# Raph1821/Matcha-TTS-etu-UPMC-ENSAM

Hardware: AMD Instinct MI355X
Metric: training utterances/sec (whole node) + maximum_path Mcells/sec, LJSpeech batch=32 (higher is better)
Workload: dtype bf16; 1 GPU; MatchaTTS train step (encoder + MAS + CFM decoder fwd/bwd + clip + AdamW), B=32/GPU, Tx=120, Ty=600, 80 mels; model=MatchaTTS(n_vocab=150, out_channels=80, hidden_channels=192), global_batch=32, seq_len=600, text_len=120, parallelism=dp1, precision=bf16-parity, hip_graph=True, weight_planes=2, text_encoder_forward=fp32fwd (backward bf16)

## Files before the change

include/mtts_decoder.h:

```cpp
#ifndef MTTS_DECODER_H_
#define MTTS_DECODER_H_

#include <stddef.h>
#include <stdint.h>

#ifdef __cplusplus
extern "C" {
#endif

#define MTTS_PREC_FP32 0
#define MTTS_PREC_BF16 1

#define MTTS_ACT_NONE 0
#define MTTS_ACT_GELU 1
#define MTTS_ACT_DGELU 2
#define MTTS_ACT_RELU 3
#define MTTS_ACT_DRELU 4

#define MTTS_CONV_MAX_TAPS 8
#define MTTS_GEMM_GLDS 32
#define MTTS_GEMM_WREG 96

typedef struct mtts_conv_gemm_args {
    const float *A;
// ... 22 lines not shown
#define MTTS_GEMM_F_A_BF16 0x2
#define MTTS_GEMM_F_C_BF16 0x4
#define MTTS_GEMM_F_FAST_ACT 0x8
#define MTTS_GEMM_F_PRE_BF16 0x10
#define MTTS_GEMM_F_W_SPLIT 0x40
#define MTTS_GEMM_F_A_SPLIT 0x80

#define MTTS_GEMM_F_SPLIT3 0x100

int mtts_conv_gemm(const mtts_conv_gemm_args *args, int32_t precision, void *hip_stream);
int mtts_conv_gemm_tile(const mtts_conv_gemm_args *args, int32_t precision, int32_t tile_cfg, void *hip_stream);
size_t mtts_conv_gemm_workspace_size(const mtts_conv_gemm_args *args, int32_t precision, int32_t tile_cfg,
                                     int32_t splits);
int mtts_conv_gemm_ws(const mtts_conv_gemm_args *args, int32_t precision, int32_t tile_cfg, int32_t splits,
                      void *workspace, size_t workspace_bytes, void *hip_stream);

typedef struct mtts_conv_wgrad_args {
    const float *dY;
    int32_t ldy, To_full, out_stride, out_off;
    const float *A;
    const float *a_scale;
    int32_t lda, Ti, To, nb, in_stride, ntaps;
    int32_t off[MTTS_CONV_MAX_TAPS];
    int32_t cin;
    int32_t N, K;
    int32_t flags;
} mtts_conv_wgrad_args;
#define MTTS_WGRAD_F_DY_BF16 0x20

size_t mtts_conv_wgrad_workspace_size(const mtts_conv_wgrad_args *args);
// ... 155 lines not shown
```

matcha-tts-etu-upmc-ensam_amd/csrc/conv_gemm.hip:

```cpp
#include <hip/hip_runtime.h>

#include <algorithm>
#include <atomic>
#include <cstdio>
#include <cstdlib>
#include <mutex>
#include <vector>

#include <cstdint>

#include "gemm_epilogue.h"
#include "conv_gemm_wreg.h"
#include "mtts_common.h"
#include "mtts_decoder.h"

namespace {

typedef __bf16 bf16x8 __attribute__((ext_vector_type(8)));
typedef float f32x16 __attribute__((ext_vector_type(16)));
typedef short s16x4 __attribute__((ext_vector_type(4)));
typedef short s16x8 __attribute__((ext_vector_type(8)));

__device__ __forceinline__ bf16x8 tr_read8(const uint16_t *p, int row_stride) {
    using LdsS4 = __attribute__((address_space(3))) s16x4;
// ... 839 lines not shown
        case 9: launch_cfg<BF16, 9>(p, M, st, splits, part); break;
        case 10: launch_cfg<BF16, 10>(p, M, st, splits, part); break;
        case 11: launch_cfg<BF16, 11>(p, M, st, splits, part); break;
        case 12: launch_cfg<BF16, 12>(p, M, st, splits, part); break;
        case 13: launch_cfg<BF16, 13>(p, M, st, splits, part); break;
        case 14: launch_cfg<BF16, 14>(p, M, st, splits, part); break;
        case 15: launch_cfg<BF16, 15>(p, M, st, splits, part); break;
        case 16: launch_cfg<BF16, 16>(p, M, st, splits, part); break;
        case 17: launch_cfg<BF16, 17>(p, M, st, splits, part); break;
        default: launch_cfg<BF16, 18>(p, M, st, splits, part); break;
    }
}

static int glds_tiles(const mtts_conv_gemm_args &p, int M) { return ((M + 63) / 64) * ((p.N + 255) / 256); }

static int pick_cfg(const mtts_conv_gemm_args &p, int M, bool bf16) {
    static const int d2 = [] { const char *e = getenv("MTTS_GEMM_F32_DEPTH2"); return e ? (e[0] == '1' ? 1 : 0) : -1; }();
    if (!bf16) return M <= 8192 ? (d2 == 1 ? 18 : 3) : (d2 == 0 ? 7 : 11);
    if (p.act == MTTS_ACT_GELU || p.act == MTTS_ACT_DGELU) return 7;
    static const int sched_mask = [] {
        const char *e = getenv("MTTS_GEMM_SCHED_OFF");
        return e ? atoi(e) : 0;
    }();
    if ((sched_mask & 4) && mtts::conv_gemm_glds_applies(p) && p.K >= 512) {
        const int t = ((M + 127) / 128) * ((p.N + 255) / 256);
        if (t >= 128 && t <= 256) return MTTS_GEMM_GLDS + 14;
    }
    if (!(sched_mask & 2) && mtts::conv_gemm_glds_applies(p) && p.K >= 768) {
        const int t = glds_tiles(p, M);
        if ((t >= 128 && t <= 256) || (t < 128 && p.K >= 1536 && p.N % 4 == 0)) return MTTS_GEMM_GLDS + 10;
        if (!(sched_mask & 8) && t > 256 && mtts::conv_gemm_glds_lean(p)) return MTTS_GEMM_GLDS + 13;
    }
    if (!(sched_mask & 8) && p.K < 768 && p.N >= 512 && glds_tiles(p, M) >= 256 && mtts::conv_gemm_glds_applies(p) &&
        mtts::conv_gemm_glds_lean(p))
        return MTTS_GEMM_GLDS + 9;
    return p.K >= 384 ? 12 : 7;
}

static int pick_cfg_a16(const mtts_conv_gemm_args &p, int M) {
    if (p.act == MTTS_ACT_GELU || p.act == MTTS_ACT_DGELU) return MTTS_GEMM_GLDS + 12;
    return glds_tiles(p, M) >= 256 ? MTTS_GEMM_GLDS + 9 : MTTS_GEMM_GLDS + 12;
}

static int pick_cfg_ws(const mtts_conv_gemm_args &p, int M) {
    if (p.act == MTTS_ACT_GELU || p.act == MTTS_ACT_DGELU) return 7;
    if (!mtts::conv_gemm_glds_applies(p) || !mtts::conv_gemm_glds_lean(p)) return 7;
    const bool big = M >= 16384 && p.N <= 256;
    if (p.flags & MTTS_GEMM_F_A_BF16) return big ? MTTS_GEMM_GLDS + 12 : MTTS_GEMM_GLDS + 9;
    return M >= 16384 ? MTTS_GEMM_GLDS + 13 : MTTS_GEMM_GLDS + 9;
}

static int pick_splits_f32(const mtts_conv_gemm_args &p, int M, int cfg, int splits) {
    static const bool off = [] { const char *e = getenv("MTTS_GEMM_F32_SPLITK"); return e && e[0] == '0'; }();
    if (p.N % 4 || off || !mtts::gemm_epilogue_vec_ok(p)) return 1;
    if (splits > 0) return splits;
    const int nk = (p.K + kBK - 1) / kBK;
    if (cfg == 3 || cfg == 18) {
        const int tiles = ((M + 63) / 64) * ((p.N + 63) / 64);
        if (tiles >= 256 || nk < 20) return 1;
        return nk >= 28 ? 4 : 2;
    }
    if (cfg != 7 && cfg != 11) return 1;
    const int tiles = ((M + 31) / 32) * ((p.N + 127) / 128);
    if (tiles >= 256 || nk < 16) return 1;
// ... 155 lines not shown
    return conv_gemm_impl(args, precision, -1, 1, nullptr, 0, hip_stream);
}

extern "C" int mtts_conv_gemm_tile(const mtts_conv_gemm_args *args, int32_t precision, int32_t tile_cfg,
                                   void *hip_stream) {
    return conv_gemm_impl(args, precision, tile_cfg, 1, nullptr, 0, hip_stream);
}

extern "C" size_t mtts_conv_gemm_workspace_size(const mtts_conv_gemm_args *args, int32_t precision, int32_t tile_cfg,
                                                int32_t splits) {
    if (!args || args->nb * args->To == 0) return 0;
    const bool bf16 = precision == MTTS_PREC_BF16;
    int rc = MTTS_OK;
    const int cfg = resolve_cfg(*args, bf16, tile_cfg, args->nb * args->To, &rc);
    return rc ? 0 : plan_gemm(*args, bf16, cfg, splits).ws;
}

extern "C" int mtts_conv_gemm_ws(const mtts_conv_gemm_args *args, int32_t precision, int32_t tile_cfg, int32_t splits,
                                 void *workspace, size_t workspace_bytes, void *hip_stream) {
    return conv_gemm_impl(args, precision, tile_cfg, splits, workspace, workspace_bytes, hip_stream);
}

__global__ void dropout_apply_kernel(const float *__restrict__ x, float *__restrict__ y, int rows, int cols, int ld,
                                     float p, const uint32_t *__restrict__ seed) {
    const int64_t idx = (int64_t)blockIdx.x * blockDim.x + threadIdx.x;
    if (idx >= (int64_t)rows * cols) return;
    const uint32_t s0 = seed[0], s1 = seed[1];
    const int r = (int)(idx / cols), c = (int)(idx - (int64_t)r * cols);
    const float v = x[(size_t)r * ld + c];
    y[(size_t)r * ld + c] = mtts::dropout_keep(s0, s1, (uint32_t)r, (uint32_t)c, p) ? v * mtts::dropout_scale(p) : 0.f;
// ... 341 lines not shown
```

matcha-tts-etu-upmc-ensam_amd/csrc/conv_gemm_glds.hip:

```cpp
#include <hip/hip_runtime.h>

#include <cstdint>
#include <type_traits>
#include <utility>

#include "gemm_epilogue.h"
#include "lds_dma.h"
#include "mtts_common.h"
#include "mtts_decoder.h"

namespace {

typedef __bf16 bf16x8 __attribute__((ext_vector_type(8)));
typedef float f32x2 __attribute__((ext_vector_type(2)));
typedef __bf16 bf16x2 __attribute__((ext_vector_type(2)));
using mtts::f32x16;

__device__ uint4 g_zero16 = {0u, 0u, 0u, 0u};

#ifndef MTTS_GEMM_TIMELINE
#define MTTS_GEMM_TIMELINE 0
#endif
#if MTTS_GEMM_TIMELINE
constexpr int kTlSlots = 128, kTlWaves = 16384, kTlSteps = 60;
// ... 12 lines not shown
constexpr int kBK = 64;

__device__ __forceinline__ uint32_t pack2(float a, float b) {
    return __builtin_bit_cast(uint32_t, __builtin_convertvector((f32x2){a, b}, bf16x2));
}

using mtts::bload16;
using mtts::glds16;
using mtts::make_rsrc;
using mtts::u32x4;
using mtts::wait_vmcnt;
constexpr uint32_t MTTS_GLDS_OOB = mtts::kDmaOob;

template <int WM, int WN, int TM, int TN, int STAGES, bool ABF16 = false, int NPL = 1>
struct GldsGeom {
    static constexpr int NT = 64 * WM * WN;
    static constexpr int BM = 32 * WM * TM, BN = 32 * WN * TN;
    static constexpr int A_BYTES = BM * kBK * (ABF16 ? 2 : 4);
    static constexpr int W_BYTES = NPL * BN * kBK * 2;
    static constexpr int GA = A_BYTES / (NT * 16);
    static constexpr int GW = W_BYTES / (NT * 16);
    static_assert(A_BYTES % (NT * 16) == 0 && W_BYTES % (NT * 16) == 0, "tile / threads mismatch");
};

template <int WM, int WN, int TM, int TN, int STAGES, bool ABF16, bool LEAN, bool WS = false, bool X3 = false>
__global__ __launch_bounds__(64 * WM * WN) void conv_gemm_glds_kernel(mtts_conv_gemm_args p, int ksteps, float *part) {
    static_assert(!X3 || (!ABF16 && !WS), "bf16x6: fp32 A, three weight planes");
    constexpr int NPL = X3 ? 3 : (WS ? 2 : 1);
    using G = GldsGeom<WM, WN, TM, TN, STAGES, ABF16, NPL>;
    constexpr int ES = ABF16 ? 2 : 4;
    constexpr int RPI = ABF16 ? 8 : 4;
    constexpr int CPR = ABF16 ? 8 : 16;
    constexpr int EPC = 16 / ES;
    constexpr int NT = G::NT, BM = G::BM, BN = G::BN, GA = G::GA, GW = G::GW, NW = NT / 64;
    __shared__ __attribute__((aligned(1024))) unsigned char sA0[G::A_BYTES], sW0[G::W_BYTES];
    __shared__ __attribute__((aligned(1024))) unsigned char sA1[G::A_BYTES], sW1[G::W_BYTES];
    __shared__ __attribute__((aligned(1024))) unsigned char sA2[STAGES > 2 ? G::A_BYTES : 16],
        sW2[STAGES > 2 ? G::W_BYTES : 16];
    auto abuf = [&](auto S) -> unsigned char * {
        if constexpr (decltype(S)::value == 0) return sA0;
        else if constexpr (decltype(S)::value == 1) return sA1;
        else return sA2;
    };
    auto wbuf = [&](auto S) -> unsigned char * {
        if constexpr (decltype(S)::value == 0) return sW0;
        else if constexpr (decltype(S)::value == 1) return sW1;
        else return sW2;
    };
    typedef __attribute__((address_space(3))) unsigned char lds_u8;
    auto lds_addr = [](const lds_u8 *q) { return (uint32_t)(uintptr_t)q; };
    auto abuf_l = [&](auto S) -> uint32_t {
        if constexpr (decltype(S)::value == 0) return lds_addr((const lds_u8 *)sA0);
        else if constexpr (decltype(S)::value == 1) return lds_addr((const lds_u8 *)sA1);
        else return lds_addr((const lds_u8 *)sA2);
    };
    auto wbuf_l = [&](auto S) -> uint32_t {
        if constexpr (decltype(S)::value == 0) return lds_addr((const lds_u8 *)sW0);
        else if constexpr (decltype(S)::value == 1) return lds_addr((const lds_u8 *)sW1);
        else return lds_addr((const lds_u8 *)sW2);
    };

    const int tid = threadIdx.x, lane = tid & 63;
    const int wave = __builtin_amdgcn_readfirstlane(tid >> 6);
    const int wr = wave / WN, wc = wave % WN;
    const int lr = lane & 31, lh = lane >> 5;
    const int M = p.nb * p.To;
    int m0, n0, kstep0 = 0, nk = (p.K + kBK - 1) / kBK;
    {
        const int nt = (p.N + BN - 1) / BN;
        const int ntiles = ((M + BM - 1) / BM) * nt;
        const int S = gridDim.x / ntiles;
        int t = mtts::xcd_relabel(blockIdx.x, gridDim.x);
        if (S > 1) {
            const int tile = t / S, split = t - tile * S;
            t = tile;
            kstep0 = split * ksteps;
            nk = min(ksteps, nk - kstep0);
        }
        const int mt = t / nt;
        m0 = mt * BM;
        n0 = (t - mt * nt) * BN;
// ... 72 lines not shown
            const int ni = 8 * (i * NW + wave) + (lane >> 3);
            const int pl = NPL > 1 ? ni / BN : 0;
            const int n = ni - pl * BN;
            const int lc = (lane & 7) ^ ((ni >> 1) & 7);
            l_vw[i] = w_nok[i] ? (uint32_t)((pl * w_plane + (size_t)(n0 + n) * p.Kp + lc * 8) * 2) : MTTS_GLDS_OOB;
        }
    }

    auto issue = [&](auto S) {
        unsigned char *abase = abuf(S);
        unsigned char *wbase = wbuf(S);
        if constexpr (LEAN) {
            const uint32_t la = abuf_l(S), lw = wbuf_l(S);
#pragma unroll
            for (int i = 0; i < GA; ++i)
                bload16(l_vo[i], l_rsa, l_soa, __builtin_amdgcn_readfirstlane(la + (i * NW + wave) * 1024));
#pragma unroll
            for (int i = 0; i < GW; ++i)
                bload16(l_vw[i], l_rsw, l_sow, __builtin_amdgcn_readfirstlane(lw + (i * NW + wave) * 1024));
            l_sow += kBK * 2;
            l_soa += kBK * ES;
            if (--l_chs == 0) {
                ++l_tap;
                l_chs = p.cin / kBK;
                l_soa = 0;
#pragma unroll
                for (int i = 0; i < GA; ++i)
                    l_vo[i] = ((a_ok[i] >> min(l_tap, 31)) & 1u) ? (uint32_t)((l_row[i] + l_tap * tapstride) * ES)
                                                                 : MTTS_GLDS_OOB;
            }
            return;
        }
#pragma unroll
        for (int i = 0; i < GA; ++i) {
            const bool ok = (a_ok[i] >> min(a_j[i], 31)) & 1u;
            glds16(ok ? static_cast<const void *>(a_src[i]) : static_cast<const void *>(zero),
                   abase + (i * NW + wave) * 1024);
            a_ch[i] += kBK;
            a_src[i] += kBK * ES;
            const bool w = a_ch[i] >= p.cin;
            a_ch[i] -= w ? p.cin : 0;
            a_j[i] += w;
            a_src[i] += w ? tap_delta : 0;
        }
#pragma unroll
        for (int i = 0; i < GW; ++i) {
            const bool ok = w_nok[i] && w_k[i] < p.Kp;
            glds16(ok ? static_cast<const void *>(w_ptr[i]) : static_cast<const void *>(zero),
                   wbase + (i * NW + wave) * 1024);
            w_ptr[i] += kBK;
            w_k[i] += kBK;
        }
    };

    f32x16 acc[TM][TN];
#pragma unroll
    for (int i = 0; i < TM; ++i)
#pragma unroll
        for (int j = 0; j < TN; ++j)
#pragma unroll
            for (int v = 0; v < 16; ++v) acc[i][j][v] = 0.f;

    auto compute = [&](auto S) {
        const unsigned char *abase = abuf(S);
// ... 89 lines not shown
#pragma unroll
                    for (int j = 0; j < TN; ++j)
                        acc[i][j] = __builtin_amdgcn_mfma_f32_32x32x16_bf16(af[i], bfr[j], acc[i][j], 0, 0, 0);
            }
        }
    };

#if MTTS_GEMM_TIMELINE
    if (lane == 0 && (int)blockIdx.x * NW + wave < kTlWaves)
        g_tlg[((int)blockIdx.x * NW + wave) * kTlSlots] =
            ((long long)__smid() << 32) | (long long)__builtin_amdgcn_s_getreg((31 << 11) | 4);
    MTTS_TLG(1);
#endif
    issue(std::integral_constant<int, 0>{});
    if constexpr (STAGES > 2) issue(std::integral_constant<int, 1>{});
    MTTS_TLG(2);
    int tl_k = 0;
    (void)tl_k;
    auto step = [&](auto S) {
        constexpr int cur = decltype(S)::value, nxt = (cur + STAGES - 1) % STAGES;
        wait_vmcnt<(GA + GW) * (STAGES - 2)>();
        mtts::lds_barrier();
#if MTTS_GEMM_TIMELINE
        if (tl_k < kTlSteps) MTTS_TLG(3 + 2 * tl_k);
#endif
        issue(std::integral_constant<int, nxt>{});
        compute(S);
#if MTTS_GEMM_TIMELINE
        __builtin_amdgcn_sched_barrier(0);
        if (tl_k < kTlSteps) MTTS_TLG(4 + 2 * tl_k);
        ++tl_k;
#endif
    };
    for (int kt = 0; kt < nk; kt += STAGES) {
        step(std::integral_constant<int, 0>{});
        if (kt + 1 >= nk) break;
        step(std::integral_constant<int, 1>{});
        if constexpr (STAGES > 2) {
            if (kt + 2 >= nk) break;
            step(std::integral_constant<int, 2>{});
        }
    }
    wait_vmcnt<0>();
    MTTS_TLG(kTlSlots - 2);
    if (part || mtts::gemm_epilogue_vec_ok(p)) {
        mtts::lds_barrier();
        unsigned char *stage = wave % 4 == 0 ? sA0 : wave % 4 == 1 ? sW0 : wave % 4 == 2 ? sA1 : sW1;
        float *st = reinterpret_cast<float *>(stage + (wave / 4) * 4096);
        if (part)
            mtts::gemm_store_partial<TM, TN>(p, acc, st, part + (size_t)(kstep0 / ksteps) * M * p.N,
                                             m0 + wr * 32 * TM, n0 + wc * 32 * TN, lane);
        else
            mtts::gemm_epilogue_vec<TM, TN>(p, acc, st, m0 + wr * 32 * TM, n0 + wc * 32 * TN, lane);
    } else {
        mtts::gemm_epilogue<TM, TN>(p, acc, m0 + wr * 32 * TM, n0 + wc * 32 * TN, lr, lh);
    }
    MTTS_TLG(kTlSlots - 1);
}

__global__ __launch_bounds__(256) void splitk_epilogue_kernel(mtts_conv_gemm_args p, const float *__restrict__ part,
                                                              int S) {
    const int M = p.nb * p.To, n4 = p.N >> 2;
    const long long idx = (long long)blockIdx.x * 256 + threadIdx.x;
// ... 8 lines not shown
    float4 bn = make_float4(0.f, 0.f, 0.f, 0.f);
    if (p.bias) bn = *reinterpret_cast<const float4 *>(p.bias + n);
    float e[4] = {a.x + bn.x, a.y + bn.y, a.z + bn.z, a.w + bn.w};
    int b, u;
    mtts::divmod_fast(m, p.To, 1.0f / (float)p.To, b, u);
    uint32_t s0 = 0, s1 = 0;
    float keep = 1.f;
    if (p.dropout_p > 0.f) {
        s0 = p.seed[0];
        s1 = p.seed[1];
        keep = mtts::dropout_scale(p.dropout_p);
    }
    mtts::epilogue_row4(p, b * p.To_full + u * p.out_stride + p.out_off, n, e, s0, s1, keep);
}

struct GldsCfg {
    int wm, wn, tm, tn, stages;
    bool f32a, bf16a;
};
constexpr GldsCfg kGlds[] = {
    {1, 4, 2, 2, 2, true, false},
    {1, 4, 2, 2, 3, false, false},
    {2, 2, 2, 2, 2, true, false},
    {2, 2, 2, 2, 3, false, false},
    {1, 4, 1, 2, 2, true, false},
    {1, 4, 1, 2, 3, true, false},
    {2, 2, 1, 2, 2, true, false},
    {2, 2, 1, 2, 3, true, false},
    {1, 4, 1, 1, 3, true, false},
    {2, 4, 1, 2, 2, true, true},
    {2, 4, 1, 2, 3, true, true},
    {1, 2, 2, 2, 3, true, false},
    {2, 2, 1, 1, 3, true, true},
    {2, 2, 1, 1, 2, true, false},
    {2, 4, 2, 2, 2, true, true},
    {4, 2, 1, 2, 2, true, false},
};
constexpr int kNumGlds = sizeof(kGlds) / sizeof(kGlds[0]);

}

namespace mtts {
bool conv_gemm_glds_lean(const mtts_conv_gemm_args &p) {
    static const bool off = [] {
        const char *e = getenv("MTTS_GLDS_LEAN");
        return e && e[0] == '0';
    }();
    const int es = (p.flags & MTTS_GEMM_F_A_BF16) ? 2 : 4;
    return !off && p.cin % kBK == 0 && (long long)p.nb * p.Ti * p.lda * es < (1ll << 31) &&
           (long long)p.N * p.Kp * 2 < (1ll << 31);
}
}

namespace {

template <int C, bool ABF16, bool WS = false, bool X3 = false>
int launch_glds_t(const mtts_conv_gemm_args &p, int M, int splits, float *part, hipStream_t st) {
    constexpr GldsCfg c = kGlds[C];
    using G = GldsGeom<c.wm, c.wn, c.tm, c.tn, c.stages, ABF16, X3 ? 3 : (WS ? 2 : 1)>;
    static_assert((!WS && !X3) || c.stages * (G::A_BYTES + G::W_BYTES) <= 160 * 1024, "split-weight stages fit LDS");
    auto kern = mtts::conv_gemm_glds_lean(p) ? conv_gemm_glds_kernel<c.wm, c.wn, c.tm, c.tn, c.stages, ABF16, true, WS, X3>
                                : conv_gemm_glds_kernel<c.wm, c.wn, c.tm, c.tn, c.stages, ABF16, false, WS, X3>;
    const int nk = (p.K + kBK - 1) / kBK;
    const int ksteps = (nk + splits - 1) / splits;
    const int S = splits > 1 ? (nk + ksteps - 1) / ksteps : 1;
    dim3 grid((unsigned)(((M + G::BM - 1) / G::BM) * ((p.N + G::BN - 1) / G::BN) * S));
    hipLaunchKernelGGL(kern, grid, dim3(G::NT), 0, st, p, ksteps, S > 1 ? part : nullptr);
    int rc = mtts::check_launch("conv_gemm_glds");
    if (rc || S == 1) return rc;
    const long long n4 = (long long)M * (p.N / 4);
    hipLaunchKernelGGL(splitk_epilogue_kernel, dim3((unsigned)((n4 + 255) / 256)), dim3(256), 0, st, p,
                       (const float *)part, S);
    return mtts::check_launch("splitk_epilogue_kernel");
}

template <int C>
int launch_glds_ws(const mtts_conv_gemm_args &p, int M, int splits, float *part, hipStream_t st) {
    constexpr int W = kGlds[C].wn * kGlds[C].tn * 32 >= 128 ? 9 : (kGlds[C].stages == 2 ? 13 : 12);
    if (p.flags & MTTS_GEMM_F_A_BF16) {
        if constexpr (kGlds[W].bf16a) return launch_glds_t<W, true, true>(p, M, splits, part, st);
        else return launch_glds_t<9, true, true>(p, M, splits, part, st);
    }
    return launch_glds_t<W, false, true>(p, M, splits, part, st);
}

template <int C>
int launch_glds_x3(const mtts_conv_gemm_args &p, int M, int splits, float *part, hipStream_t st) {
    if constexpr (kGlds[C].stages >= 3) return launch_glds_t<12, false, false, true>(p, M, splits, part, st);
    else return launch_glds_t<13, false, false, true>(p, M, splits, part, st);
}

template <int C>
int launch_glds(const mtts_conv_gemm_args &p, int M, int splits, float *part, hipStream_t st) {
    if (p.flags & MTTS_GEMM_F_SPLIT3) return launch_glds_x3<C>(p, M, splits, part, st);
    if (p.flags & MTTS_GEMM_F_W_SPLIT) return launch_glds_ws<C>(p, M, splits, part, st);
    if (p.flags & MTTS_GEMM_F_A_BF16) {
        if constexpr (kGlds[C].bf16a) return launch_glds_t<C, true>(p, M, splits, part, st);
        else return launch_glds_t<9, true>(p, M, splits, part, st);
    }
    if constexpr (kGlds[C].f32a) return launch_glds_t<C, false>(p, M, splits, part, st);
    else return launch_glds_t<9, false>(p, M, splits, part, st);
}

template <int... I>
int launch_glds_id(int id, const mtts_conv_gemm_args &p, int M, int splits, float *part, hipStream_t st,
                   std::integer_sequence<int, I...>) {
    int rc = MTTS_ERR_INVALID_ARG;
    ((id == I ? (rc = launch_glds<I>(p, M, splits, part, st), true) : false) || ...);
    return rc;
}

}

namespace mtts {

int conv_gemm_glds_num_cfgs() { return kNumGlds; }
// ... 12 lines not shown
    const int nk = (p.K + kBK - 1) / kBK;
    const int ksteps = (nk + splits - 1) / splits;
    const int S = (nk + ksteps - 1) / ksteps;
    return S > 1 ? (size_t)S * p.nb * p.To * p.N * sizeof(float) : 0;
}

int splitk_combine(const mtts_conv_gemm_args &p, int M, const float *part, int S, hipStream_t st) {
    const long long n4 = (long long)M * (p.N / 4);
    hipLaunchKernelGGL(splitk_epilogue_kernel, dim3((unsigned)((n4 + 255) / 256)), dim3(256), 0, st, p, part, S);
    return mtts::check_launch("splitk_epilogue_kernel");
}

int conv_gemm_glds_launch(int id, const mtts_conv_gemm_args &p, int M, int splits, float *part, hipStream_t st) {
    return launch_glds_id(id, p, M, splits, part, st, std::make_integer_sequence<int, kNumGlds>{});
}
}

#if MTTS_GEMM_TIMELINE
extern "C" long long mtts_glds_timeline_read(void *host) {
    const size_t bytes = sizeof(long long) * kTlWaves * kTlSlots;
    if (host) {
        if (hipMemcpyFromSymbol(host, HIP_SYMBOL(g_tlg), bytes) != hipSuccess) return -1;
    } else {
        void *d = nullptr;
        if (hipGetSymbolAddress(&d, HIP_SYMBOL(g_tlg)) != hipSuccess || hipMemset(d, 0, bytes) != hipSuccess) return -1;
    }
    return (long long)bytes;
}
#endif
```

matcha-tts-etu-upmc-ensam_amd/csrc/mtts_common.h:

```cpp
#pragma once

#include <hip/hip_runtime.h>

#include <cstdint>

#include "mtts_base.h"
#include "mtts_decoder.h"

namespace mtts {

__device__ __forceinline__ bool dropout_keep(uint32_t seed_lo, uint32_t seed_hi, uint32_t row, uint32_t col,
                                             float p) {
    uint32_t x = ((row * 0x9E3779B1u) ^ (((col >> 1) + 0x7F4A7C15u) * 0x85EBCA77u) ^ seed_lo) + seed_hi;
    x ^= x >> 16; x *= 0x85EBCA6Bu; x ^= x >> 13; x *= 0xC2B2AE35u; x ^= x >> 16;
    const uint32_t u = (col & 1u) ? (x >> 16) : (x & 0xFFFFu);
    return (float)u * (1.0f / 65536.0f) >= p;
}

__host__ __device__ __forceinline__ float dropout_scale(float p) {
    return p > 0.f ? 65536.0f / (65536.0f - ceilf(p * 65536.0f)) : 1.0f;
}

template <class P>
__device__ __forceinline__ int tap_off(const P &p, int j) {
    int o = p.off[0];
#pragma unroll
    for (int i = 1; i < MTTS_CONV_MAX_TAPS; ++i) o = j == i ? p.off[i] : o;
    return o;
}

}

struct mtts_conv_gemm_args;
namespace mtts {
int conv_gemm_glds_num_cfgs();
bool conv_gemm_glds_applies(const mtts_conv_gemm_args &p);
bool conv_gemm_glds_lean(const mtts_conv_gemm_args &p);
int conv_gemm_glds_launch(int id, const mtts_conv_gemm_args &p, int M, int splits, float *part, hipStream_t st);
size_t conv_gemm_glds_splitk_bytes(const mtts_conv_gemm_args &p, int splits);
}

struct mtts_reduce_job;
namespace mtts {
int submit_reductions(const mtts_reduce_job *jobs, int njobs, hipStream_t st);
int queue_reductions(const mtts_reduce_job *jobs, int njobs);
bool deferring();
int flush_wgrads(hipStream_t st);
int pending_wgrad_sums();
void discard_wgrads();
}
```

matcha-tts-etu-upmc-ensam_amd/matcha/_native.py:

```python
from __future__ import annotations

import ctypes
import os
from pathlib import Path

import torch

_PKG_ROOT = Path(__file__).resolve().parent.parent
LIB_PATH = Path(os.environ.get("MTTS_LIB", _PKG_ROOT / "lib" / "libmtts_hip.so"))

MTTS_OK = 0
MTTS_MAS_VALUE_PREMASKED = 0x1
MTTS_MAS_NO_DENSE_PATH = 0x2
MTTS_MAS_MAX_TX = 8192
MTTS_MAS_MAX_TX_ROW_MAJOR = 4096

_P = ctypes.c_void_p
_I32 = ctypes.c_int32
_I64 = ctypes.c_int64
_F = ctypes.c_float
_SZ = ctypes.c_size_t

_SIGNATURES: dict[str, tuple] = {
    "mtts_abi_version": (ctypes.c_int, []),
# ... 4 lines not shown
    "mtts_prior_maximum_path": (ctypes.c_int, [_P, _P, _P, _P, _I32, _I32, _I32, _I32, _P, _P, _P, _P, _P, _P, _P,
                                               _SZ, _P]),
    "mtts_expand_rows_fwd": (ctypes.c_int, [_P, _P, _I32, _I32, _I32, _I32, _P, _P]),
    "mtts_expand_rows_bwd": (ctypes.c_int, [_P, _P, _P, _I32, _I32, _I32, _I32, _P, _P]),
    "mtts_segment_crop_fwd": (ctypes.c_int, [_P, _P, _P, _P, _P, _P, _I32, _I32, _I32, _I32, _I32, _P, _P, _P, _P, _P,
                                             _P]),
    "mtts_segment_crop_bwd": (ctypes.c_int, [_P, _P, _P, _P, _I32, _I32, _I32, _I32, _P, _P]),
    "mtts_compute_batch_alignments": (ctypes.c_int, [_P, _P, _P, _P, _I32, _I32, _I32, _F, _P, _SZ, _P]),
    "mtts_losses_workspace_size": (_SZ, [_I32, _I32]),
    "mtts_losses_fwd": (ctypes.c_int, [_P, _P, _P, _P, _P, _P, _I32, _I32, _I32, _F, _P, _P, _SZ, _P]),
    "mtts_losses_bwd": (ctypes.c_int, [_P, _P, _P, _P, _P, _P, _P, _P, _P, _I32, _I32, _I32, _F, _P, _P, _P]),
    "mtts_cfm_pack_fwd": (ctypes.c_int, [_P, _P, _P, _P, _I32, _I32, _I32, _F, _P, _P]),
    "mtts_cfm_pack_bwd": (ctypes.c_int, [_P, _I32, _I32, _I32, _P, _P]),
    "mtts_time_embedding": (ctypes.c_int, [_P, _I32, _I32, _F, _P, _P]),
    "mtts_mel_log_fwd": (ctypes.c_int, [_P, _P, _P, _P, _I32, _I32, _I32, _I32, _F, _P, _P]),
}

_lib = None


class NativeError(RuntimeError):
    pass


def register(name: str, restype, argtypes) -> None:
    _SIGNATURES[name] = (restype, argtypes)
    if _lib is not None:
        _bind(_lib, name)


# ... 39 lines not shown
```

Measured before the change: 4358 utterances/s.

## Pick GLDS GEMM tile by occupancy-rounds cost model and add 10-wave/4-stage tiles

Replaces the hand-written GLDS tile heuristics for the bf16 GEMM paths (plain, bf16-A and split-weight workspace) with a small cost model. The model counts wave rounds from LDS-limited residency and adds an estimated stage-fill time, then takes the cheapest among the candidate configs. The kernel template now supports ragged per-wave DMA distribution (tile sizes not divisible by wave count) and up to four stages, which enables new 5x2-wave configs. The config table is reorganized by kind bitmask, and new plan/occupancy query entry points are exported. Risks: the cost-model constants are rough, so it may pick slower tiles for some shapes, and the ragged-wait logic adds complexity.

After: 4486 utterances/s, median of 6. +2.9%, better.

```diff
diff --git a/include/mtts_decoder.h b/include/mtts_decoder.h
--- a/include/mtts_decoder.h
+++ b/include/mtts_decoder.h
@@ -60,6 +60,9 @@
                                      int32_t splits);
 int mtts_conv_gemm_ws(const mtts_conv_gemm_args *args, int32_t precision, int32_t tile_cfg, int32_t splits,
                       void *workspace, size_t workspace_bytes, void *hip_stream);
+int mtts_conv_gemm_plan(const mtts_conv_gemm_args *args, int32_t precision, int32_t tile_cfg, int32_t splits,
+                        int32_t out[6]);
+int mtts_conv_gemm_glds_occupancy(int32_t schedule, int32_t kind, int32_t lean, int32_t out[2]);
 
 typedef struct mtts_conv_wgrad_args {
     const float *dY;
diff --git a/matcha-tts-etu-upmc-ensam_amd/csrc/conv_gemm.hip b/matcha-tts-etu-upmc-ensam_amd/csrc/conv_gemm.hip
--- a/matcha-tts-etu-upmc-ensam_amd/csrc/conv_gemm.hip
+++ b/matcha-tts-etu-upmc-ensam_amd/csrc/conv_gemm.hip
@@ -877,24 +877,51 @@
 
 static int glds_tiles(const mtts_conv_gemm_args &p, int M) { return ((M + 63) / 64) * ((p.N + 255) / 256); }
 
+struct GldsRounds {
+    int tiles, resident, rounds, fill_pm;
+    double us;
+};
+constexpr double kGldsFixedUs = 3.5, kGldsFillBps = 65e9;
+static GldsRounds glds_rounds(const mtts_conv_gemm_args &p, int M, int id, int splits) {
+    const mtts::GldsInfo g = mtts::conv_gemm_glds_info(id, p);
+    GldsRounds r = {};
+    if (g.resident < 1) return r;
+    const int nk = (p.K + 63) / 64, ksteps = splits > 1 ? (nk + splits - 1) / splits : nk;
+    const int S = splits > 1 ? (nk + ksteps - 1) / ksteps : 1;
+    const int slots = 256 * g.resident;
+    r.tiles = ((M + g.bm - 1) / g.bm) * ((p.N + g.bn - 1) / g.bn) * S;
+    r.resident = g.resident;
+    r.rounds = (r.tiles + slots - 1) / slots;
+    r.fill_pm = (int)((1000ll * r.tiles) / ((long long)r.rounds * slots));
+    r.us = r.rounds * kGldsFixedUs + (double)((r.tiles + 255) / 256) * ksteps * g.stage_bytes / kGldsFillBps * 1e6;
+    return r;
+}
+
+static int pick_glds_rounds(const mtts_conv_gemm_args &p, int M) {
+    static const int kPickable[] = {14, 15, 9, 10, 12, 13};
+    if (!(p.flags & (MTTS_GEMM_F_A_BF16 | MTTS_GEMM_F_W_SPLIT)) && glds_tiles(p, M) > 256) return MTTS_GEMM_GLDS + 13;
+    int best = -1;
+    double best_us = 0.;
+    for (int id : kPickable) {
+        if (!mtts::conv_gemm_glds_info(id, p).own) continue;
+        const GldsRounds r = glds_rounds(p, M, id, 1);
+        if (r.resident < 1) continue;
+        if (best < 0 || r.us < best_us) best = id, best_us = r.us;
+    }
+    return MTTS_GEMM_GLDS + best;
+}
+
 static int pick_cfg(const mtts_conv_gemm_args &p, int M, bool bf16) {
     static const int d2 = [] { const char *e = getenv("MTTS_GEMM_F32_DEPTH2"); return e ? (e[0] == '1' ? 1 : 0) : -1; }();
     if (!bf16) return M <= 8192 ? (d2 == 1 ? 18 : 3) : (d2 == 0 ? 7 : 11);
     if (p.act == MTTS_ACT_GELU || p.act == MTTS_ACT_DGELU) return 7;
-    static const int sched_mask = [] {
-        const char *e = getenv("MTTS_GEMM_SCHED_OFF");
-        return e ? atoi(e) : 0;
-    }();
-    if ((sched_mask & 4) && mtts::conv_gemm_glds_applies(p) && p.K >= 512) {
-        const int t = ((M + 127) / 128) * ((p.N + 255) / 256);
-        if (t >= 128 && t <= 256) return MTTS_GEMM_GLDS + 14;
-    }
-    if (!(sched_mask & 2) && mtts::conv_gemm_glds_applies(p) && p.K >= 768) {
+    if (mtts::conv_gemm_glds_applies(p) && p.K >= 768) {
         const int t = glds_tiles(p, M);
-        if ((t >= 128 && t <= 256) || (t < 128 && p.K >= 1536 && p.N % 4 == 0)) return MTTS_GEMM_GLDS + 10;
-        if (!(sched_mask & 8) && t > 256 && mtts::conv_gemm_glds_lean(p)) return MTTS_GEMM_GLDS + 13;
-    }
-    if (!(sched_mask & 8) && p.K < 768 && p.N >= 512 && glds_tiles(p, M) >= 256 && mtts::conv_gemm_glds_applies(p) &&
+        if (t < 128 && p.K >= 1536 && p.N % 4 == 0) return MTTS_GEMM_GLDS + 10;
+        if (t >= 128 && mtts::conv_gemm_glds_lean(p)) return pick_glds_rounds(p, M);
+        if (t >= 128 && t <= 256) return MTTS_GEMM_GLDS + 10;
+    }
+    if (p.K < 768 && p.N >= 512 && glds_tiles(p, M) >= 256 && mtts::conv_gemm_glds_applies(p) &&
         mtts::conv_gemm_glds_lean(p))
         return MTTS_GEMM_GLDS + 9;
     return p.K >= 384 ? 12 : 7;
@@ -902,15 +929,14 @@
 
 static int pick_cfg_a16(const mtts_conv_gemm_args &p, int M) {
     if (p.act == MTTS_ACT_GELU || p.act == MTTS_ACT_DGELU) return MTTS_GEMM_GLDS + 12;
+    if (mtts::conv_gemm_glds_lean(p)) return pick_glds_rounds(p, M);
     return glds_tiles(p, M) >= 256 ? MTTS_GEMM_GLDS + 9 : MTTS_GEMM_GLDS + 12;
 }
 
 static int pick_cfg_ws(const mtts_conv_gemm_args &p, int M) {
     if (p.act == MTTS_ACT_GELU || p.act == MTTS_ACT_DGELU) return 7;
     if (!mtts::conv_gemm_glds_applies(p) || !mtts::conv_gemm_glds_lean(p)) return 7;
-    const bool big = M >= 16384 && p.N <= 256;
-    if (p.flags & MTTS_GEMM_F_A_BF16) return big ? MTTS_GEMM_GLDS + 12 : MTTS_GEMM_GLDS + 9;
-    return M >= 16384 ? MTTS_GEMM_GLDS + 13 : MTTS_GEMM_GLDS + 9;
+    return pick_glds_rounds(p, M);
 }
 
 static int pick_splits_f32(const mtts_conv_gemm_args &p, int M, int cfg, int splits) {
@@ -1096,6 +1122,28 @@
     int rc = MTTS_OK;
     const int cfg = resolve_cfg(*args, bf16, tile_cfg, args->nb * args->To, &rc);
     return rc ? 0 : plan_gemm(*args, bf16, cfg, splits).ws;
+}
+
+extern "C" int mtts_conv_gemm_plan(const mtts_conv_gemm_args *args, int32_t precision, int32_t tile_cfg,
+                                   int32_t splits, int32_t out[6]) {
+    MTTS_CHECK_ARG(args && out, "conv_gemm_plan: null argument");
+    MTTS_CHECK_ARG(precision == MTTS_PREC_BF16 || precision == MTTS_PREC_FP32, "conv_gemm_plan: bad precision");
+    MTTS_CHECK_ARG(splits >= 0, "conv_gemm_plan: bad split count");
+    const bool bf16 = precision == MTTS_PREC_BF16;
+    const int M = args->nb * args->To;
+    int rc = MTTS_OK;
+    const int cfg = resolve_cfg(*args, bf16, tile_cfg, M, &rc);
+    if (rc) return rc;
+    const GemmPlan pl = plan_gemm(*args, bf16, cfg, splits);
+    GldsRounds r = {};
+    int s = pl.splits;
+    if (pl.cfg >= MTTS_GEMM_GLDS && pl.cfg < MTTS_GEMM_WREG) {
+        if (pl.ws == 0) s = 1;
+        r = glds_rounds(*args, M, pl.cfg - MTTS_GEMM_GLDS, s);
+        if (s > 1) s = (int)(pl.ws / ((size_t)M * args->N * sizeof(float)));
+    }
+    out[0] = pl.cfg, out[1] = s, out[2] = r.tiles, out[3] = r.resident, out[4] = r.rounds, out[5] = r.fill_pm;
+    return MTTS_OK;
 }
 
 extern "C" int mtts_conv_gemm_ws(const mtts_conv_gemm_args *args, int32_t precision, int32_t tile_cfg, int32_t splits,
diff --git a/matcha-tts-etu-upmc-ensam_amd/csrc/conv_gemm_glds.hip b/matcha-tts-etu-upmc-ensam_amd/csrc/conv_gemm_glds.hip
--- a/matcha-tts-etu-upmc-ensam_amd/csrc/conv_gemm_glds.hip
+++ b/matcha-tts-etu-upmc-ensam_amd/csrc/conv_gemm_glds.hip
@@ -50,13 +50,19 @@
 
 template <int WM, int WN, int TM, int TN, int STAGES, bool ABF16 = false, int NPL = 1>
 struct GldsGeom {
-    static constexpr int NT = 64 * WM * WN;
+    static constexpr int NT = 64 * WM * WN, NW = WM * WN;
     static constexpr int BM = 32 * WM * TM, BN = 32 * WN * TN;
     static constexpr int A_BYTES = BM * kBK * (ABF16 ? 2 : 4);
     static constexpr int W_BYTES = NPL * BN * kBK * 2;
-    static constexpr int GA = A_BYTES / (NT * 16);
-    static constexpr int GW = W_BYTES / (NT * 16);
-    static_assert(A_BYTES % (NT * 16) == 0 && W_BYTES % (NT * 16) == 0, "tile / threads mismatch");
+    static constexpr int NIA = A_BYTES / 1024, NIW = W_BYTES / 1024;
+    static constexpr int GA = (NIA + NW - 1) / NW, GW = (NIW + NW - 1) / NW;
+    static constexpr int RA = NIA % NW, RW = NIW % NW;
+    static constexpr bool RAGGED = RA != 0 || RW != 0;
+    static_assert(A_BYTES % 1024 == 0 && W_BYTES % 1024 == 0, "whole DMA instructions");
+    static_assert(STAGES >= 2 && STAGES <= 4, "two to four stage buffers");
+    static constexpr int SA = A_BYTES / 4096, SW = W_BYTES / 4096;
+    static_assert(NW <= 8 ? (SA >= (NW + 3) / 4 && SW >= (NW + 2) / 4) : 2 * (SA + SW) >= NW,
+                  "the epilogue's per-wave staging images fit the stage buffers");
 };
 
 template <int WM, int WN, int TM, int TN, int STAGES, bool ABF16, bool LEAN, bool WS = false, bool X3 = false>
@@ -68,32 +74,38 @@
     constexpr int RPI = ABF16 ? 8 : 4;
     constexpr int CPR = ABF16 ? 8 : 16;
     constexpr int EPC = 16 / ES;
-    constexpr int NT = G::NT, BM = G::BM, BN = G::BN, GA = G::GA, GW = G::GW, NW = NT / 64;
+    constexpr int NT = G::NT, BM = G::BM, BN = G::BN, GA = G::GA, GW = G::GW, NW = G::NW;
     __shared__ __attribute__((aligned(1024))) unsigned char sA0[G::A_BYTES], sW0[G::W_BYTES];
     __shared__ __attribute__((aligned(1024))) unsigned char sA1[G::A_BYTES], sW1[G::W_BYTES];
     __shared__ __attribute__((aligned(1024))) unsigned char sA2[STAGES > 2 ? G::A_BYTES : 16],
         sW2[STAGES > 2 ? G::W_BYTES : 16];
+    __shared__ __attribute__((aligned(1024))) unsigned char sA3[STAGES > 3 ? G::A_BYTES : 16],
+        sW3[STAGES > 3 ? G::W_BYTES : 16];
     auto abuf = [&](auto S) -> unsigned char * {
         if constexpr (decltype(S)::value == 0) return sA0;
         else if constexpr (decltype(S)::value == 1) return sA1;
-        else return sA2;
+        else if constexpr (decltype(S)::value == 2) return sA2;
+        else return sA3;
     };
     auto wbuf = [&](auto S) -> unsigned char * {
         if constexpr (decltype(S)::value == 0) return sW0;
         else if constexpr (decltype(S)::value == 1) return sW1;
-        else return sW2;
+        else if constexpr (decltype(S)::value == 2) return sW2;
+        else return sW3;
     };
     typedef __attribute__((address_space(3))) unsigned char lds_u8;
     auto lds_addr = [](const lds_u8 *q) { return (uint32_t)(uintptr_t)q; };
     auto abuf_l = [&](auto S) -> uint32_t {
         if constexpr (decltype(S)::value == 0) return lds_addr((const lds_u8 *)sA0);
         else if constexpr (decltype(S)::value == 1) return lds_addr((const lds_u8 *)sA1);
-        else return lds_addr((const lds_u8 *)sA2);
+        else if constexpr (decltype(S)::value == 2) return lds_addr((const lds_u8 *)sA2);
+        else return lds_addr((const lds_u8 *)sA3);
     };
     auto wbuf_l = [&](auto S) -> uint32_t {
         if constexpr (decltype(S)::value == 0) return lds_addr((const lds_u8 *)sW0);
         else if constexpr (decltype(S)::value == 1) return lds_addr((const lds_u8 *)sW1);
-        else return lds_addr((const lds_u8 *)sW2);
+        else if constexpr (decltype(S)::value == 2) return lds_addr((const lds_u8 *)sW2);
+        else return lds_addr((const lds_u8 *)sW3);
     };
 
     const int tid = threadIdx.x, lane = tid & 63;
@@ -101,6 +113,7 @@
     const int wr = wave / WN, wc = wave % WN;
     const int lr = lane & 31, lh = lane >> 5;
     const int M = p.nb * p.To;
+    const bool a_last = G::RA == 0 || wave < G::RA, w_last = G::RW == 0 || wave < G::RW;
     int m0, n0, kstep0 = 0, nk = (p.K + kBK - 1) / kBK;
     {
         const int nt = (p.N + BN - 1) / BN;
@@ -203,10 +216,12 @@
             const uint32_t la = abuf_l(S), lw = wbuf_l(S);
 #pragma unroll
             for (int i = 0; i < GA; ++i)
-                bload16(l_vo[i], l_rsa, l_soa, __builtin_amdgcn_readfirstlane(la + (i * NW + wave) * 1024));
+                if (i < GA - 1 || a_last)
+                    bload16(l_vo[i], l_rsa, l_soa, __builtin_amdgcn_readfirstlane(la + (i * NW + wave) * 1024));
 #pragma unroll
             for (int i = 0; i < GW; ++i)
-                bload16(l_vw[i], l_rsw, l_sow, __builtin_amdgcn_readfirstlane(lw + (i * NW + wave) * 1024));
+                if (i < GW - 1 || w_last)
+                    bload16(l_vw[i], l_rsw, l_sow, __builtin_amdgcn_readfirstlane(lw + (i * NW + wave) * 1024));
             l_sow += kBK * 2;
             l_soa += kBK * ES;
             if (--l_chs == 0) {
@@ -223,8 +238,9 @@
 #pragma unroll
         for (int i = 0; i < GA; ++i) {
             const bool ok = (a_ok[i] >> min(a_j[i], 31)) & 1u;
-            glds16(ok ? static_cast<const void *>(a_src[i]) : static_cast<const void *>(zero),
-                   abase + (i * NW + wave) * 1024);
+            if (i < GA - 1 || a_last)
+                glds16(ok ? static_cast<const void *>(a_src[i]) : static_cast<const void *>(zero),
+                       abase + (i * NW + wave) * 1024);
             a_ch[i] += kBK;
             a_src[i] += kBK * ES;
             const bool w = a_ch[i] >= p.cin;
@@ -235,8 +251,9 @@
 #pragma unroll
         for (int i = 0; i < GW; ++i) {
             const bool ok = w_nok[i] && w_k[i] < p.Kp;
-            glds16(ok ? static_cast<const void *>(w_ptr[i]) : static_cast<const void *>(zero),
-                   wbase + (i * NW + wave) * 1024);
+            if (i < GW - 1 || w_last)
+                glds16(ok ? static_cast<const void *>(w_ptr[i]) : static_cast<const void *>(zero),
+                       wbase + (i * NW + wave) * 1024);
             w_ptr[i] += kBK;
             w_k[i] += kBK;
         }
@@ -356,12 +373,21 @@
 #endif
     issue(std::integral_constant<int, 0>{});
     if constexpr (STAGES > 2) issue(std::integral_constant<int, 1>{});
+    if constexpr (STAGES > 3) issue(std::integral_constant<int, 2>{});
     MTTS_TLG(2);
     int tl_k = 0;
     (void)tl_k;
     auto step = [&](auto S) {
         constexpr int cur = decltype(S)::value, nxt = (cur + STAGES - 1) % STAGES;
-        wait_vmcnt<(GA + GW) * (STAGES - 2)>();
+        constexpr int F = (GA + GW) * (STAGES - 2);
+        if constexpr (!G::RAGGED || STAGES == 2) {
+            wait_vmcnt<F>();
+        } else {
+            const int less = (a_last ? 0 : 1) + (w_last ? 0 : 1);
+            if (less == 0) wait_vmcnt<F>();
+            else if (less == 1) wait_vmcnt<F - (STAGES - 2)>();
+            else wait_vmcnt<F - 2 * (STAGES - 2)>();
+        }
         mtts::lds_barrier();
 #if MTTS_GEMM_TIMELINE
         if (tl_k < kTlSteps) MTTS_TLG(3 + 2 * tl_k);
@@ -382,13 +408,26 @@
             if (kt + 2 >= nk) break;
             step(std::integral_constant<int, 2>{});
         }
+        if constexpr (STAGES > 3) {
+            if (kt + 3 >= nk) break;
+            step(std::integral_constant<int, 3>{});
+        }
     }
     wait_vmcnt<0>();
     MTTS_TLG(kTlSlots - 2);
     if (part || mtts::gemm_epilogue_vec_ok(p)) {
         mtts::lds_barrier();
-        unsigned char *stage = wave % 4 == 0 ? sA0 : wave % 4 == 1 ? sW0 : wave % 4 == 2 ? sA1 : sW1;
-        float *st = reinterpret_cast<float *>(stage + (wave / 4) * 4096);
+        unsigned char *stage;
+        if constexpr (NW <= 8) {
+            stage = (wave % 4 == 0 ? sA0 : wave % 4 == 1 ? sW0 : wave % 4 == 2 ? sA1 : sW1) + (wave / 4) * 4096;
+        } else {
+            constexpr int SA = G::SA, SW = G::SW;
+            stage = wave < SA ? sA0 + wave * 4096
+                    : wave < SA + SW ? sW0 + (wave - SA) * 4096
+                    : wave < 2 * SA + SW ? sA1 + (wave - SA - SW) * 4096
+                                         : sW1 + (wave - 2 * SA - SW) * 4096;
+        }
+        float *st = reinterpret_cast<float *>(stage);
         if (part)
             mtts::gemm_store_partial<TM, TN>(p, acc, st, part + (size_t)(kstep0 / ksteps) * M * p.N,
                                              m0 + wr * 32 * TM, n0 + wc * 32 * TN, lane);
@@ -427,29 +466,61 @@
     mtts::epilogue_row4(p, b * p.To_full + u * p.out_stride + p.out_off, n, e, s0, s1, keep);
 }
 
+enum : unsigned { kF32 = 1u, kB16 = 2u, kF32WS = 4u, kB16WS = 8u, kX3 = 16u };
+constexpr int kNumKinds = 5;
+constexpr bool kind_a16(int kind) { return kind == 1 || kind == 3; }
+constexpr int kind_planes(int kind) { return kind == 4 ? 3 : kind >= 2 ? 2 : 1; }
+inline int kind_of(const mtts_conv_gemm_args &p) {
+    if (p.flags & MTTS_GEMM_F_SPLIT3) return 4;
+    return ((p.flags & MTTS_GEMM_F_W_SPLIT) ? 2 : 0) + ((p.flags & MTTS_GEMM_F_A_BF16) ? 1 : 0);
+}
+
 struct GldsCfg {
     int wm, wn, tm, tn, stages;
-    bool f32a, bf16a;
+    unsigned kinds;
+    bool lean_only = false;
 };
 constexpr GldsCfg kGlds[] = {
-    {1, 4, 2, 2, 2, true, false},
-    {1, 4, 2, 2, 3, false, false},
-    {2, 2, 2, 2, 2, true, false},
-    {2, 2, 2, 2, 3, false, false},
-    {1, 4, 1, 2, 2, true, false},
-    {1, 4, 1, 2, 3, true, false},
-    {2, 2, 1, 2, 2, true, false},
-    {2, 2, 1, 2, 3, true, false},
-    {1, 4, 1, 1, 3, true, false},
-    {2, 4, 1, 2, 2, true, true},
-    {2, 4, 1, 2, 3, true, true},
-    {1, 2, 2, 2, 3, true, false},
-    {2, 2, 1, 1, 3, true, true},
-    {2, 2, 1, 1, 2, true, false},
-    {2, 4, 2, 2, 2, true, true},
-    {4, 2, 1, 2, 2, true, false},
+    {1, 4, 2, 2, 2, kF32},
+    {1, 4, 2, 2, 3, 0},
+    {2, 2, 2, 2, 2, kF32},
+    {2, 2, 2, 2, 3, 0},
+    {1, 4, 1, 2, 2, kF32},
+    {1, 4, 1, 2, 3, kF32},
+    {2, 2, 1, 2, 2, kF32},
+    {2, 2, 1, 2, 3, kF32},
+    {1, 4, 1, 1, 3, kF32},
+    {2, 4, 1, 2, 2, kF32 | kB16 | kF32WS | kB16WS},
+    {2, 4, 1, 2, 3, kF32 | kB16},
+    {1, 2, 2, 2, 3, kF32},
+    {2, 2, 1, 1, 3, kF32 | kB16 | kF32WS | kB16WS | kX3},
+    {2, 2, 1, 1, 2, kF32 | kF32WS | kX3},
+    {5, 2, 1, 1, 2, kF32 | kB16 | kF32WS | kB16WS},
+    {5, 2, 1, 2, 3, kB16 | kB16WS, true},
 };
 constexpr int kNumGlds = sizeof(kGlds) / sizeof(kGlds[0]);
+
+constexpr int glds_run_id(int c, int kind, bool lean = true) {
+    if (kGlds[c].lean_only && !lean) return 9;
+    if (kGlds[c].kinds & (1u << kind)) return c;
+    if (kind == 4) return kGlds[c].stages >= 3 ? 12 : 13;
+    if (kind >= 2) {
+        const int w = kGlds[c].wn * kGlds[c].tn * 32 >= 128 ? 9 : (kGlds[c].stages == 2 ? 13 : 12);
+        return (kGlds[w].kinds & (1u << kind)) ? w : 9;
+    }
+    return 9;
+}
+constexpr int glds_bm(int c) { return 32 * kGlds[c].wm * kGlds[c].tm; }
+constexpr int glds_bn(int c) { return 32 * kGlds[c].wn * kGlds[c].tn; }
+constexpr int glds_stage_bytes(int c, int kind) {
+    return glds_bm(c) * kBK * (kind_a16(kind) ? 2 : 4) + kind_planes(kind) * glds_bn(c) * kBK * 2;
+}
+constexpr int glds_resident(int c, int kind, bool lean = true) {
+    if (c == 9 && kind == 1 && !lean) return 1;
+    const int lds = kGlds[c].stages * glds_stage_bytes(c, kind), nt = 64 * kGlds[c].wm * kGlds[c].wn;
+    const int by_lds = 160 * 1024 / lds, by_thr = 2048 / nt;
+    return by_lds < by_thr ? by_lds : by_thr;
+}
 
 }
 
@@ -467,18 +538,29 @@
 
 namespace {
 
-template <int C, bool ABF16, bool WS = false, bool X3 = false>
+template <int C, int KIND>
+auto glds_kernel(bool lean) {
+    constexpr GldsCfg c = kGlds[C];
+    constexpr bool A16 = kind_a16(KIND), WS = KIND == 2 || KIND == 3, X3 = KIND == 4;
+    if constexpr (c.lean_only) {
+        return conv_gemm_glds_kernel<c.wm, c.wn, c.tm, c.tn, c.stages, A16, true, WS, X3>;
+    } else {
+        return lean ? conv_gemm_glds_kernel<c.wm, c.wn, c.tm, c.tn, c.stages, A16, true, WS, X3>
+                    : conv_gemm_glds_kernel<c.wm, c.wn, c.tm, c.tn, c.stages, A16, false, WS, X3>;
+    }
+}
+
+template <int C, int KIND>
 int launch_glds_t(const mtts_conv_gemm_args &p, int M, int splits, float *part, hipStream_t st) {
-    constexpr GldsCfg c = kGlds[C];
-    using G = GldsGeom<c.wm, c.wn, c.tm, c.tn, c.stages, ABF16, X3 ? 3 : (WS ? 2 : 1)>;
-    static_assert((!WS && !X3) || c.stages * (G::A_BYTES + G::W_BYTES) <= 160 * 1024, "split-weight stages fit LDS");
-    auto kern = mtts::conv_gemm_glds_lean(p) ? conv_gemm_glds_kernel<c.wm, c.wn, c.tm, c.tn, c.stages, ABF16, true, WS, X3>
-                                : conv_gemm_glds_kernel<c.wm, c.wn, c.tm, c.tn, c.stages, ABF16, false, WS, X3>;
+    static_assert(kGlds[C].kinds & (1u << KIND), "an instantiated kind");
+    static_assert(glds_resident(C, KIND) >= 1, "the stages fit LDS");
+    constexpr int BM = glds_bm(C), BN = glds_bn(C), NT = 64 * kGlds[C].wm * kGlds[C].wn;
+    auto kern = glds_kernel<C, KIND>(mtts::conv_gemm_glds_lean(p));
     const int nk = (p.K + kBK - 1) / kBK;
     const int ksteps = (nk + splits - 1) / splits;
     const int S = splits > 1 ? (nk + ksteps - 1) / ksteps : 1;
-    dim3 grid((unsigned)(((M + G::BM - 1) / G::BM) * ((p.N + G::BN - 1) / G::BN) * S));
-    hipLaunchKernelGGL(kern, grid, dim3(G::NT), 0, st, p, ksteps, S > 1 ? part : nullptr);
+    dim3 grid((unsigned)(((M + BM - 1) / BM) * ((p.N + BN - 1) / BN) * S));
+    hipLaunchKernelGGL(kern, grid, dim3(NT), 0, st, p, ksteps, S > 1 ? part : nullptr);
     int rc = mtts::check_launch("conv_gemm_glds");
     if (rc || S == 1) return rc;
     const long long n4 = (long long)M * (p.N / 4);
@@ -488,31 +570,46 @@
 }
 
 template <int C>
-int launch_glds_ws(const mtts_conv_gemm_args &p, int M, int splits, float *part, hipStream_t st) {
-    constexpr int W = kGlds[C].wn * kGlds[C].tn * 32 >= 128 ? 9 : (kGlds[C].stages == 2 ? 13 : 12);
-    if (p.flags & MTTS_GEMM_F_A_BF16) {
-        if constexpr (kGlds[W].bf16a) return launch_glds_t<W, true, true>(p, M, splits, part, st);
-        else return launch_glds_t<9, true, true>(p, M, splits, part, st);
-    }
-    return launch_glds_t<W, false, true>(p, M, splits, part, st);
+int launch_glds(const mtts_conv_gemm_args &p, int M, int splits, float *part, hipStream_t st) {
+    if constexpr (kGlds[C].lean_only) {
+        if (!mtts::conv_gemm_glds_lean(p)) return launch_glds<9>(p, M, splits, part, st);
+    }
+    switch (kind_of(p)) {
+        case 4: return launch_glds_t<glds_run_id(C, 4), 4>(p, M, splits, part, st);
+        case 3: return launch_glds_t<glds_run_id(C, 3), 3>(p, M, splits, part, st);
+        case 2: return launch_glds_t<glds_run_id(C, 2), 2>(p, M, splits, part, st);
+        case 1: return launch_glds_t<glds_run_id(C, 1), 1>(p, M, splits, part, st);
+        default: return launch_glds_t<glds_run_id(C, 0), 0>(p, M, splits, part, st);
+    }
 }
 
 template <int C>
-int launch_glds_x3(const mtts_conv_gemm_args &p, int M, int splits, float *part, hipStream_t st) {
-    if constexpr (kGlds[C].stages >= 3) return launch_glds_t<12, false, false, true>(p, M, splits, part, st);
-    else return launch_glds_t<13, false, false, true>(p, M, splits, part, st);
-}
-
-template <int C>
-int launch_glds(const mtts_conv_gemm_args &p, int M, int splits, float *part, hipStream_t st) {
-    if (p.flags & MTTS_GEMM_F_SPLIT3) return launch_glds_x3<C>(p, M, splits, part, st);
-    if (p.flags & MTTS_GEMM_F_W_SPLIT) return launch_glds_ws<C>(p, M, splits, part, st);
-    if (p.flags & MTTS_GEMM_F_A_BF16) {
-        if constexpr (kGlds[C].bf16a) return launch_glds_t<C, true>(p, M, splits, part, st);
-        else return launch_glds_t<9, true>(p, M, splits, part, st);
-    }
-    if constexpr (kGlds[C].f32a) return launch_glds_t<C, false>(p, M, splits, part, st);
-    else return launch_glds_t<9, false>(p, M, splits, part, st);
+int occupancy_glds(int kind, bool lean) {
+    int n = -1;
+    auto ask = [&](auto K) {
+        constexpr int KIND = decltype(K)::value;
+        if constexpr ((kGlds[C].kinds & (1u << KIND)) != 0) {
+            if (hipOccupancyMaxActiveBlocksPerMultiprocessor(&n, glds_kernel<C, KIND>(lean), 64 * kGlds[C].wm * kGlds[C].wn,
+                                                             0) != hipSuccess)
+                n = -2;
+        }
+    };
+    switch (kind) {
+        case 0: ask(std::integral_constant<int, 0>{}); break;
+        case 1: ask(std::integral_constant<int, 1>{}); break;
+        case 2: ask(std::integral_constant<int, 2>{}); break;
+        case 3: ask(std::integral_constant<int, 3>{}); break;
+        case 4: ask(std::integral_constant<int, 4>{}); break;
+        default: break;
+    }
+    return n;
+}
+
+template <int... I>
+int occupancy_glds_id(int id, int kind, bool lean, std::integer_sequence<int, I...>) {
+    int n = -1;
+    ((id == I ? (n = occupancy_glds<I>(kind, lean), true) : false) || ...);
+    return n;
 }
 
 template <int... I>
@@ -555,6 +652,32 @@
 int conv_gemm_glds_launch(int id, const mtts_conv_gemm_args &p, int M, int splits, float *part, hipStream_t st) {
     return launch_glds_id(id, p, M, splits, part, st, std::make_integer_sequence<int, kNumGlds>{});
 }
+
+GldsInfo conv_gemm_glds_info(int id, const mtts_conv_gemm_args &p) {
+    const int kind = kind_of(p);
+    GldsInfo g = {};
+    if (id < 0 || id >= kNumGlds) return g;
+    const int r = glds_run_id(id, kind, conv_gemm_glds_lean(p));
+    g.run_id = r;
+    g.bm = glds_bm(r);
+    g.bn = glds_bn(r);
+    g.stages = kGlds[r].stages;
+    g.stage_bytes = glds_stage_bytes(r, kind);
+    g.resident = glds_resident(r, kind, conv_gemm_glds_lean(p));
+    g.own = r == id;
+    return g;
+}
+}
+
+extern "C" int mtts_conv_gemm_glds_occupancy(int32_t schedule, int32_t kind, int32_t lean, int32_t out[2]) {
+    const int id = schedule - MTTS_GEMM_GLDS;
+    MTTS_CHECK_ARG(out && id >= 0 && id < kNumGlds && kind >= 0 && kind < kNumKinds &&
+                       (kGlds[id].kinds & (1u << kind)) && (lean || !kGlds[id].lean_only),
+                   "conv_gemm_glds_occupancy: no such instantiation");
+    out[0] = glds_resident(id, kind, lean != 0);
+    out[1] = occupancy_glds_id(id, kind, lean != 0, std::make_integer_sequence<int, kNumGlds>{});
+    if (out[1] < 0) return mtts::fail(MTTS_ERR_HIP, "conv_gemm_glds_occupancy: occupancy query failed");
+    return MTTS_OK;
 }
 
 #if MTTS_GEMM_TIMELINE
diff --git a/matcha-tts-etu-upmc-ensam_amd/csrc/mtts_common.h b/matcha-tts-etu-upmc-ensam_amd/csrc/mtts_common.h
--- a/matcha-tts-etu-upmc-ensam_amd/csrc/mtts_common.h
+++ b/matcha-tts-etu-upmc-ensam_amd/csrc/mtts_common.h
@@ -38,6 +38,14 @@
 bool conv_gemm_glds_lean(const mtts_conv_gemm_args &p);
 int conv_gemm_glds_launch(int id, const mtts_conv_gemm_args &p, int M, int splits, float *part, hipStream_t st);
 size_t conv_gemm_glds_splitk_bytes(const mtts_conv_gemm_args &p, int splits);
+struct GldsInfo {
+    int run_id;
+    int bm, bn, stages;
+    int stage_bytes;
+    int resident;
+    bool own;
+};
+GldsInfo conv_gemm_glds_info(int id, const mtts_conv_gemm_args &p);
 }
 
 struct mtts_reduce_job;
diff --git a/matcha-tts-etu-upmc-ensam_amd/matcha/_native.py b/matcha-tts-etu-upmc-ensam_amd/matcha/_native.py
--- a/matcha-tts-etu-upmc-ensam_amd/matcha/_native.py
+++ b/matcha-tts-etu-upmc-ensam_amd/matcha/_native.py
@@ -42,6 +42,8 @@
     "mtts_cfm_pack_bwd": (ctypes.c_int, [_P, _I32, _I32, _I32, _P, _P]),
     "mtts_time_embedding": (ctypes.c_int, [_P, _I32, _I32, _F, _P, _P]),
     "mtts_mel_log_fwd": (ctypes.c_int, [_P, _P, _P, _P, _I32, _I32, _I32, _I32, _F, _P, _P]),
+    "mtts_conv_gemm_plan": (ctypes.c_int, [_P, _I32, _I32, _I32, ctypes.POINTER(_I32 * 6)]),
+    "mtts_conv_gemm_glds_occupancy": (ctypes.c_int, [_I32, _I32, _I32, ctypes.POINTER(_I32 * 2)]),
 }
 
 _lib = None
```
